# Bergvca/string_grouper

Hardware: AMD Instinct MI355X
Metric: hot-path rows/sec (the device path of match_strings: tokenise + tf-idf + postings + SpGEMM-topn, inputs resident in HBM), 663k-name self-join ntop=10 min_sim=0.8; match_strings end to end: match_strings_rows_per_s (higher is better)
Workload: dtype f32

## Files before the change

string_grouper_amd/csrc/sg_k4_device.h:

```cpp
#ifndef SG_K4_DEVICE_H
#define SG_K4_DEVICE_H
#include <math.h>

#include "sg_internal.h"

#define SG_TOPN_LANES 64

#ifdef SG_WATCHDOG
static __device__ int g_sg_watch[4];
#define SG_WD_DECL(c) int c = 0
#define SG_WD(c, limit, code)                                   \
    if (++(c) > (int)(limit) || ((volatile int *)g_sg_watch)[0]) { \
        if (((volatile int *)g_sg_watch)[0] == 0) {             \
            g_sg_watch[0] = (code);                             \
            g_sg_watch[1] = (int)(c);                           \
        }                                                       \
        break;                                                  \
    }
#ifndef SG_WATCH_NAME
#define SG_WATCH_NAME sg_debug_watch
#endif
extern "C" int SG_WATCH_NAME(int32_t *out4) {
    return hipMemcpyFromSymbol(out4, HIP_SYMBOL(g_sg_watch), 16) == hipSuccess ? 0 : 4;
}
// ... 45 lines not shown
    int c;
    __device__ __forceinline__ void clear() {
        s = -INFINITY;
        c = INT32_MAX;
    }
    __device__ __forceinline__ void insert(T ns, int nc, int lane) {
        const bool mine_first = (s > ns) || (s == ns && c < nc);
        const int pos = __popcll(__ballot(mine_first));
        if (pos >= SG_TOPN_LANES) return;
        const T us = __shfl_up(s, 1, 64);
        const int uc = __shfl_up(c, 1, 64);
        if (lane > pos) {
            s = us;
            c = uc;
        } else if (lane == pos) {
            s = ns;
            c = nc;
        }
    }
    __device__ __forceinline__ void insert_unique(T ns, int nc, int lane) {
        if (__ballot(c == nc) != 0) return;
        insert(ns, nc, lane);
    }
};

template <typename T>
struct TopListWide {
    TopList<T> lo, hi;
    __device__ __forceinline__ void clear() {
        lo.clear();
        hi.clear();
    }
    __device__ __forceinline__ void insert(T ns, int nc, int lane) {
        const bool mine_first = (lo.s > ns) || (lo.s == ns && lo.c < nc);
        const int pos = __popcll(__ballot(mine_first));
        if (pos >= SG_TOPN_LANES) {
            hi.insert(ns, nc, lane);
            return;
        }
        const T es = wave_read<T>(lo.s, SG_TOPN_LANES - 1);
        const int ec = wave_read<int>(lo.c, SG_TOPN_LANES - 1);
        lo.insert(ns, nc, lane);
        if (ec != INT32_MAX) hi.insert(es, ec, lane);
    }
    __device__ __forceinline__ void insert_unique(T ns, int nc, int lane) {
        if (__ballot(lo.c == nc || hi.c == nc) != 0) return;
        insert(ns, nc, lane);
    }
    __device__ __forceinline__ int count() const {
        return __popcll(__ballot(lo.c != INT32_MAX)) + __popcll(__ballot(hi.c != INT32_MAX));
    }
};

template <typename T>
struct Post;
template <>
struct Post<float> {
    typedef uint2 reg_t;
    static constexpr int STRIDE = 8;
    static __device__ __forceinline__ reg_t load(const char *vals, const char *, uint32_t seg_lo, uint32_t entry) {
        return *reinterpret_cast<const uint2 *>(vals + ((seg_lo + entry) << 3));
    }
    static __device__ __forceinline__ uint32_t slot(const reg_t &r) { return r.x; }
    static __device__ __forceinline__ float val(const reg_t &r) { return __uint_as_float(r.y); }
};
template <>
struct Post<double> {
    struct reg_t {
        uint32_t j;
        double v;
    };
    static constexpr int STRIDE = 8;
    static __device__ __forceinline__ reg_t load(const char *vals, const char *slots, uint32_t seg_lo, uint32_t entry) {
        reg_t r;
        r.j = *reinterpret_cast<const uint32_t *>(slots + ((seg_lo + entry) << 2));
        r.v = *reinterpret_cast<const double *>(vals + ((seg_lo + entry) << 3));
        return r;
    }
    static __device__ __forceinline__ uint32_t slot(const reg_t &r) { return r.j; }
    static __device__ __forceinline__ double val(const reg_t &r) { return r.v; }
};


__device__ __forceinline__ uint32_t next_row(uint32_t *row_counter, int lane) {
    uint32_t r = 0;
    if (lane == 0) r = __hip_atomic_fetch_add(row_counter, 1u, __ATOMIC_RELAXED, __HIP_MEMORY_SCOPE_AGENT);
    return (uint32_t)__builtin_amdgcn_readfirstlane((int)r);
}

#endif
```

string_grouper_amd/csrc/sg_spgemm_pruned.hip:

```cpp
#define SG_WATCH_NAME sg_debug_watch_pruned
#include "sg_k4_device.h"

#ifdef SG_DEBUG_WAVE_TIMES
__device__ unsigned long long sg_debug_wave_times[4 * 16384];
extern "C" int sg_debug_read_wave_times(unsigned long long *out, int clear) {
    if (hipMemcpyFromSymbol(out, HIP_SYMBOL(sg_debug_wave_times), sizeof(sg_debug_wave_times)) != hipSuccess) return 1;
    if (clear) {
        static unsigned long long zero[4 * 16384];
        if (hipMemcpyToSymbol(HIP_SYMBOL(sg_debug_wave_times), zero, sizeof(zero)) != hipSuccess) return 1;
    }
    return 0;
}
#endif

#ifndef SG_F64_STREAM_WAVES
#define SG_F64_STREAM_WAVES 4
#endif
#define SG_SCHED_FENCE() __builtin_amdgcn_sched_barrier(0)
#define SG_ROW_PARTS_LOG2 6
#define SG_ROW_PARTS 64u
#define SG_SURV_CAP 128

__device__ __forceinline__ uint64_t ballot64(bool p) { return __builtin_amdgcn_ballot_w64(p); }

// ... 402 lines not shown
    if ((uint32_t)lane < n_surv) {
        c0 = surv[lane];
        k0 = (uint32_t)lane < n_clean ||
             __hip_atomic_exchange(&dt[((uint32_t)c0 * 2654435761u) >> 25], (uint32_t)c0, __ATOMIC_RELAXED,
                                   __HIP_MEMORY_SCOPE_WORKGROUP) != (uint32_t)c0;
    }
    if ((uint32_t)lane + 64u < n_surv) {
        c1 = surv[lane + 64];
        k1 = (uint32_t)lane + 64u < n_clean ||
             __hip_atomic_exchange(&dt[((uint32_t)c1 * 2654435761u) >> 25], (uint32_t)c1, __ATOMIC_RELAXED,
                                   __HIP_MEMORY_SCOPE_WORKGROUP) != (uint32_t)c1;
    }
    const uint64_t f0 = ballot64(k0), f1 = ballot64(k1);
    const uint32_t n0 = (uint32_t)__popcll(f0);
    __builtin_amdgcn_wave_barrier();
    if (k0) surv[__popcll(f0 & lanes_below)] = c0;
    if (k1) surv[n0 + __popcll(f1 & lanes_below)] = c1;
    __builtin_amdgcn_wave_barrier();
    FlushOut<T> out;
    out.top = top;
    out.n_surv = (uint32_t)__builtin_amdgcn_readfirstlane((int)(n0 + (uint32_t)__popcll(f1)));
    if (out.n_surv >= 63u) {
        out.top = drain_survivors<T, SYM, TILE_LOG2, WIDE, true>(nnz, thr, row, sc, pairs, top, out.n_surv);
        const uint32_t scored = out.n_surv < 64u ? out.n_surv : 64u;
        out.n_surv = (out.n_surv - scored) | (scored << 16);
    }
    return out;
}

template <typename T, int TILE_LOG2>
__device__ __noinline__ void emit_part_matches(const SgPairSink *__restrict__ pairs, T s, int c, int cnt, uint32_t row_out) {
    constexpr int TILE = 1 << TILE_LOG2;
    int *surv = lds_object<int>(TILE * 2 + 512 + 1024);
    const int lane = threadIdx.x;
    if (cnt <= 0) return;
    uint32_t pos = (uint32_t)surv[SG_SURV_CAP - 1];
    const SgPairSink pv = load_launch_constants(pairs);
    const uint32_t pair_chunks = pv.chunks;
    if (pos == SG_PAIR_NO_CHUNK || (pos & 511u) + (uint32_t)cnt > SG_PAIR_CHUNK) {
        uint32_t ch = 0;
        if (lane == 0) {
            if (pos != SG_PAIR_NO_CHUNK && (pos >> 9) < pair_chunks) {
                pv.d_chunk_count[pos >> 9] = pos & 511u;
                atomicAdd(pv.d_totals, (unsigned long long)(pos & 511u));
            }
            ch = atomicAdd(pv.d_chunks_used, 1u);
        }
        pos = (uint32_t)__builtin_amdgcn_readfirstlane((int)ch) << 9;
    }
    if ((pos >> 9) < pair_chunks) {
        if (lane < cnt) {
            const size_t o = (size_t)(pos >> 9) * SG_PAIR_CHUNK + (pos & 511u) + (uint32_t)lane;
            pv.d_i[o] = (uint32_t)c;
            pv.d_j[o] = row_out;
            reinterpret_cast<T *>(pv.d_s)[o] = s;
        }
        if (lane == 0) atomicAdd(&pv.d_row_count[row_out], (uint32_t)cnt);
    }
    __builtin_amdgcn_wave_barrier();
    if (lane == 0) surv[SG_SURV_CAP - 1] = (int)(pos + (uint32_t)cnt);
}

template <typename T, int TILE_LOG2, bool SYM, bool WIDE, int FOLD_LOG2, bool SHARE = false>
__global__ void __launch_bounds__(64, (sizeof(T) == 8 && FOLD_LOG2 > 0) ? SG_F64_STREAM_WAVES : 4)
spgemm_topn_pruned_kernel(const int64_t *__restrict__ a_indptr, const int32_t *__restrict__ a_indices,
                          const T *__restrict__ a_data, uint32_t n_left, const uint32_t *__restrict__ seg,
                          const uint32_t *__restrict__ ends, int32_t nt_pad, uint32_t n_terms,
                          const uint32_t *__restrict__ filt, int32_t n_tiles,
                          const SgScoreCtx *__restrict__ sc ,
                          int32_t keep, int32_t out_stride, T thr,
                          float s_budget , float norm_b ,
                          uint32_t freq_min ,
                          int32_t *__restrict__ out_cols, T *__restrict__ out_vals, int32_t *__restrict__ out_cnt,
                          uint32_t *row_counter, uint32_t *flagged_count, uint32_t *flagged_rows,
                          unsigned long long *stats ,
                          const SgPairSink *__restrict__ pairs ,
                          uint32_t pair_chunks ,
                          uint32_t sym_lo, uint32_t sym_hi ,
                          const uint32_t *__restrict__ row_list , const uint32_t *row_list_len,
                          const uint32_t *__restrict__ ends8 , int32_t nv_pad,
                          uint32_t null_off ,
                          uint32_t n_right ,
                          uint32_t *heavy_count, uint32_t *heavy_rows ,
                          uint32_t sym_step,
                          uint32_t part_cfg ) {
    constexpr int TILE = 1 << TILE_LOG2;
    constexpr int SLOTS = WIDE ? 2 : 1;
    constexpr int AB = TILE_LOG2 + 1;
    constexpr uint32_t ADDR_MASK = ((1u << AB) - 1u) & ~3u;
    constexpr int FB = AB + FOLD_LOG2;
    constexpr uint32_t BQ_BITS = 24 - FB;
    constexpr uint32_t BQ_MAX = (1u << BQ_BITS) - 1u;
    constexpr float SCALE = (float)(32768 >> FOLD_LOG2);
    extern __shared__ __attribute__((aligned(16))) unsigned char smem[];
    int *hk = reinterpret_cast<int *>(smem + TILE * 2);
    T *ha = reinterpret_cast<T *>(smem + TILE * 2 + 512);
    int *surv = reinterpret_cast<int *>(smem + TILE * 2 + 512 + 1024);
    uint4 *tab_v = reinterpret_cast<uint4 *>(smem);
    const int lane = threadIdx.x;
    for (int x = lane; x < TILE * 2 / 16; x += 64) tab_v[x] = make_uint4(0, 0, 0, 0);
    if (SYM && lane == 0) surv[SG_SURV_CAP - 1] = (int)SG_PAIR_NO_CHUNK;
    if (FOLD_LOG2 > 0 && lane == 0) surv[SG_SURV_CAP - 2] = 0;
    const uint64_t lanes_below = (1ull << lane) - 1ull;
    unsigned long long st_rows = 0, st_post = 0, st_surv = 0;
    auto tab_at = [&](uint32_t byte_addr) {
        typedef __attribute__((address_space(3))) uint32_t lds_u32;
        return (uint32_t *)(lds_u32 *)(uintptr_t)byte_addr;
    };
    auto filt_at = [&](uint32_t byte_off) {
        return *reinterpret_cast<const uint32_t *>(reinterpret_cast<const char *>(filt) + byte_off);
    };

    SG_WD_DECL(wd_rows);
    constexpr bool CAN_SPLIT = SYM && !WIDE && FOLD_LOG2 > 0 && SHARE;
    const bool part_mode = CAN_SPLIT && (part_cfg >> 31) != 0u;
#ifdef SG_DEBUG_WAVE_TIMES
    const unsigned long long dbg_t0 = __builtin_amdgcn_s_memrealtime();
    unsigned long long dbg_worst = 0, dbg_worst_row = 0;
#endif
    const uint32_t n_here = (WIDE || part_mode) ? (uint32_t)__builtin_amdgcn_readfirstlane((int)*row_list_len) << (part_mode ? SG_ROW_PARTS_LOG2 : 0)
                                                : (SYM ? (sym_hi - sym_lo + sym_step - 1u) / sym_step : n_left);
    const uint32_t n_single = min(n_here, 2u * gridDim.x);
    const uint32_t n_quads = (n_here - n_single) >> 2;
    for (uint32_t hlp = next_row(row_counter, lane);; hlp = next_row(row_counter, lane)) {
    const uint32_t row0 = hlp < n_quads ? hlp << 2 : (n_quads << 2) + (hlp - n_quads);
    if (row0 >= n_here || hlp >= 0x10000000u) break;
    for (uint32_t rr = row0; rr < row0 + (hlp < n_quads ? 4u : 1u); ++rr) {
        SG_WD(wd_rows, n_left + 2, 11)
        const uint32_t row = WIDE ? (uint32_t)__builtin_amdgcn_readfirstlane((int)row_list[rr])
                                  : part_mode ? (uint32_t)__builtin_amdgcn_readfirstlane((int)row_list[rr >> SG_ROW_PARTS_LOG2])
                                              : (SYM ? sym_hi - 1u - rr * sym_step : rr);
        uint32_t part_lo = 0, part_hi = 0;
        if (CAN_SPLIT && part_mode) {
            const uint32_t from = (uint32_t)__builtin_amdgcn_readfirstlane((int)row_list[n_left + (rr >> SG_ROW_PARTS_LOG2)]);
            const uint32_t nv = (((row >> TILE_LOG2) + (1u << FOLD_LOG2)) >> FOLD_LOG2) - from;
            const uint32_t part = rr & (SG_ROW_PARTS - 1u);
            part_lo = from + ((part * nv) >> SG_ROW_PARTS_LOG2);
            part_hi = from + (((part + 1u) * nv) >> SG_ROW_PARTS_LOG2);
            if (part_lo == part_hi) continue;
        }
        uint32_t row_out = row;
        if (SYM) {
            const uint32_t *orig_of = sc->orig_of;
            if (orig_of) row_out = (uint32_t)__builtin_amdgcn_readfirstlane((int)orig_of[row]);
        }
        const int64_t rlo = a_indptr[row];
        const int nnz = __builtin_amdgcn_readfirstlane((int)(a_indptr[row + 1] - rlo));
        if (nnz > 64 * SLOTS) {
            if (lane == 0) flagged_rows[atomicAdd(flagged_count, 1u)] = row;
            continue;
        }
        if (nnz == 0) continue;
        int k[SLOTS];
        T a[SLOTS];
        uint32_t df[SLOTS], lo_e[SLOTS];
        float w[SLOTS], cum[SLOTS];
#pragma unroll
        for (int sl = 0; sl < SLOTS; ++sl) {
            k[sl] = 0;
            a[sl] = (T)0;
            df[sl] = lo_e[sl] = 0;
            if (lane + 64 * sl < nnz) {
                k[sl] = a_indices[rlo + lane + 64 * sl];
                a[sl] = a_data[rlo + lane + 64 * sl];
                const uint32_t *sp = seg + (int64_t)k[sl] * n_tiles;
                lo_e[sl] = sp[0];
                df[sl] = sp[n_tiles] - lo_e[sl];
            }
            w[sl] = lane + 64 * sl < nnz ? (float)a[sl] * (float)a[sl] * 1.00001f : 0.f;
            cum[sl] = 0.f;
        }
        for (int q = 0; q < nnz; ++q) {
            uint32_t dq;
            float wq;
            if (SLOTS == 1 || q < 64) {
                dq = wave_read<uint32_t>(df[0], q);
                wq = wave_read<float>(w[0], q);
            } else {
                dq = wave_read<uint32_t>(df[SLOTS - 1], q - 64);
                wq = wave_read<float>(w[SLOTS - 1], q - 64);
            }
#pragma unroll
            for (int sl = 0; sl < SLOTS; ++sl) {
                const bool before = dq > df[sl] || (dq == df[sl] && q <= lane + 64 * sl);
                cum[sl] += before ? wq : 0.f;
            }
        }
        bool in_p[SLOTS];
        uint64_t pm[SLOTS];
        float bs2 = 0.f, dsum = 0.f;
        int np = 0;
#pragma unroll
        for (int sl = 0; sl < SLOTS; ++sl) {
            const bool have = lane + 64 * sl < nnz;
            const bool in_s = have && cum[sl] <= s_budget && df[sl] >= freq_min;
            in_p[sl] = have && !in_s;
            pm[sl] = __ballot(in_p[sl]);
            np += __popcll(pm[sl]);
            bs2 = fmaxf(bs2, in_s ? cum[sl] : 0.f);
            dsum += in_p[sl] ? (float)df[sl] : 0.f;
        }
        if (np == 0) continue;
        if (np > 64) {
            if (lane == 0) flagged_rows[atomicAdd(flagged_count, 1u)] = row;
            continue;
        }
        if (!part_mode) ++st_rows;
#ifdef SG_DEBUG_WAVE_TIMES
        const unsigned long long dbg_r0 = __builtin_amdgcn_s_memrealtime();
        const unsigned long long dbg_surv0 = st_surv;
#endif
#pragma unroll
        for (int d = 32; d > 0; d >>= 1) {
            bs2 = fmaxf(bs2, __shfl_xor(bs2, d, 64));
            dsum += __shfl_xor(dsum, d, 64);
        }
        bs2 = wave_read<float>(bs2, 0);
        dsum = wave_read<float>(dsum, 0);
        if (!(dsum > 0.f)) continue;
        const float b_s = sqrtf(bs2) * 1.000002f;
        const float t0 = ((float)thr - 1e-5f) * SCALE - 2.0f;
        const float c1 = b_s * norm_b * (SCALE / 255.0f) * 1.000002f;
        const int32_t T0 = (int32_t)floorf(t0 * 256.0f) - 256 * np;
        const int32_t C1 = (int32_t)(c1 * 256.0f) + 1;
        const int32_t C16 = (int32_t)(b_s * norm_b * (SCALE * 65536.0f / 65280.0f) * 1.000002f) + 1;
        const int32_t T16 = T0 << 8;
        const int32_t T0s = T16 - 32768 * C16, C1n = -C16;
        if (FOLD_LOG2 > 0 ? !(T16 - C16 * 65535 >= 65536) : !(T0 - C1 * 255 >= 256)) {
            if (lane == 0) flagged_rows[atomicAdd(flagged_count, 1u)] = row;
            continue;
        }
        const int32_t T0m = T0 - 256;

        uint32_t G[SLOTS], start[SLOTS];
        uint32_t before_slot = 0;
#pragma unroll
        for (int sl = 0; sl < SLOTS; ++sl) {
            G[sl] = in_p[sl] ? 1u + (uint32_t)((float)(64 - np) * 0.999f * ((float)df[sl] / dsum)) : 0u;
            uint32_t inc = G[sl];
#pragma unroll
            for (int d = 1; d < 64; d <<= 1) {
                const uint32_t o = __shfl_up(inc, d, 64);
                if (lane >= d) inc += o;
            }
            start[sl] = before_slot + inc - G[sl];
            before_slot += wave_read<uint32_t>(inc, 63);
        }
        int src = 0, src_slot = 0;
        uint32_t u = 0, g = 0;
#pragma unroll
        for (int sl = 0; sl < SLOTS; ++sl) {
            uint64_t m = pm[sl];
            SG_WD_DECL(wd_a);
            while (m) {
                SG_WD(wd_a, 70, 12)
                const int f = __builtin_ctzll(m);
                m &= m - 1;
                const uint32_t sf = wave_read<uint32_t>(start[sl], f), gf = wave_read<uint32_t>(G[sl], f);
                const uint32_t d = (uint32_t)lane - sf;
                if (d < gf) {
                    src = f;
                    src_slot = sl;
                    u = d;
                    g = gf;
                }
            }
        }
        int my_k = wave_shfl<int>(k[0], src);
        uint32_t my_lo = wave_shfl<uint32_t>(lo_e[0], src);
        T my_a = wave_shfl<T>(a[0], src);
        if (SLOTS > 1) {
            const int k1 = wave_shfl<int>(k[SLOTS - 1], src);
            const uint32_t lo1 = wave_shfl<uint32_t>(lo_e[SLOTS - 1], src);
            const T a1 = wave_shfl<T>(a[SLOTS - 1], src);
            if (src_slot) {
                my_k = k1;
                my_lo = lo1;
                my_a = a1;
            }
        }
        const float c_a = (float)my_a * norm_b * (SCALE / (float)BQ_MAX) * 1.000002f;
        const uint32_t CA = (uint32_t)(c_a * (float)(1u << (32 - FB))) + 1u;
        const uint32_t u4 = u << 2, u16 = u << 4, G4 = g << 2, G16 = g << 4;
        const int32_t over16 = (int32_t)(G16 - u16);
        const uint32_t erow = (g ? (uint32_t)my_k : n_terms) * (uint32_t)nt_pad;
        auto ends_at = [&](uint32_t group) {
            return *reinterpret_cast<const uint4 *>(reinterpret_cast<const char *>(ends) + ((erow + (group << 2)) << 2));
        };
        const uint32_t t_end = SYM ? (row >> TILE_LOG2) + 1u : (uint32_t)n_tiles;
        const uint32_t last_group = (uint32_t)(nt_pad >> 2) - 1u;

        if (WIDE) {
#pragma unroll
            for (int sl = 0; sl < SLOTS; ++sl) {
                hk[lane + 64 * sl] = lane + 64 * sl < nnz ? k[sl] : INT32_MAX;
                ha[lane + 64 * sl] = a[sl];
            }
            __builtin_amdgcn_wave_barrier();
        } else {
            hk[lane] = -1;
            hk[lane + 64] = -1;
            __builtin_amdgcn_wave_barrier();
            if (lane < nnz) {
                uint32_t h = term_hash(k[0]);
                SG_WD_DECL(wd_i);
                while (atomicCAS(&hk[h], -1, k[0]) != -1) {
                    SG_WD(wd_i, SG_HASH_SLOTS + 2, 16)
                    h = (h + 1) & (SG_HASH_SLOTS - 1);
                }
                ha[h] = a[0];
            }
            __builtin_amdgcn_wave_barrier();
        }

        TopList<T> top;
        top.clear();
        uint32_t n_surv = 0;
        uint32_t row_arg = row | ((SYM && keep > SG_TOPN_LANES) ? 0x40000000u : 0u);
        if (SYM && FOLD_LOG2 > 0 && !part_mode) {
            T own = (T)0;
            for (int q = 0; q < nnz; ++q) {
                const T aq = (SLOTS == 1 || q < 64) ? wave_read<T>(a[0], q) : wave_read<T>(a[SLOTS - 1], q - 64);
                own = add_rn<T>(own, mul_rn<T>(aq, aq));
            }
            if (own > thr) top.insert(own, (int)row_out, lane);
            row_arg |= 0x80000000u;
        }

        auto collect = [&](uint64_t cm, uint32_t r, uint32_t t) {
            bool cross = (cm >> lane) & 1ull;
            const int col = (int)((t << TILE_LOG2) | ((r & ADDR_MASK) >> 1) | (r & 1u));
            if (SYM) {
                cross = cross && (uint32_t)col <= row;
                cm = ballot64(cross);
            }
            if (cross) surv[n_surv + __popcll(cm & lanes_below)] = col;
            n_surv += __popcll(cm);
            if (n_surv >= 64) {
                top = drain_survivors<T, SYM, TILE_LOG2, WIDE, (FOLD_LOG2 > 0)>(nnz, thr, row_arg, sc, pairs, top, n_surv);
                st_surv += 64;
                n_surv -= 64;
            }
        };
        auto round = [&](uint32_t r, bool valid, uint64_t valid_mask, uint32_t t, uint32_t &zaddr) {
            zaddr = r & ADDR_MASK;
            const uint32_t sh = r << 4;
            const uint32_t x = (uint32_t)(((uint64_t)(r & (BQ_MAX << FB)) * (uint64_t)(CA & 0xffffffu)) >> 32);
            const uint32_t tq1 = (uint32_t)((T0m - __mul24(C1, (int32_t)(r >> 24))) >> 8);
            uint32_t xs;
            asm("v_lshlrev_b32 %0, %1, %2" : "=v"(xs) : "v"(sh), "v"(x));
            uint32_t old;
            asm("" : "=v"(old));
            if (valid)
                old = __hip_atomic_fetch_add(tab_at(zaddr), xs, __ATOMIC_RELAXED, __HIP_MEMORY_SCOPE_WORKGROUP);
            asm volatile("" : "+v"(old));
            const uint32_t oh = __builtin_amdgcn_ubfe(old, sh, 16u);
            const uint64_t cm = ballot64(tq1 - oh < x) & valid_mask;
            if (cm) collect(cm, r, t);
        };

        struct Batch {
            uint32_t r0, r1, r2, r3;
            int32_t rem;
            uint32_t base;
        };
        auto issue = [&](Batch &bt, uint32_t lo, uint32_t hi) {
            bt.base = lo + u16;
            bt.rem = (int32_t)(hi - bt.base);
            struct __attribute__((packed, aligned(4))) Quad {
                uint32_t x, y, z, w;
            };
            const Quad q = *reinterpret_cast<const Quad *>(reinterpret_cast<const char *>(filt) + bt.base);
            bt.r0 = q.x;
            bt.r1 = q.y;
            bt.r2 = q.z;
            bt.r3 = q.w;
        };
        struct Slot {
            uint32_t z, sh, x, xs, tq1;
        };
        auto prep = [&](uint32_t r) {
            Slot s;
            s.z = r & ADDR_MASK;
            s.sh = r << 4;
            s.x = (uint32_t)(((uint64_t)(r & (BQ_MAX << FB)) * (uint64_t)(CA & 0xffffffu)) >> 32);
            s.tq1 = (uint32_t)((T0m - __mul24(C1, (int32_t)(r >> 24))) >> 8);
            asm("v_lshlrev_b32 %0, %1, %2" : "=v"(s.xs) : "v"(s.sh), "v"(s.x));
            return s;
        };
        auto apply = [&](const Batch &bt, uint32_t t) {
            const bool v0 = bt.rem > 0, v1 = bt.rem > 4, v2 = bt.rem > 8, v3 = bt.rem > 12;
            const uint64_t m0 = ballot64(v0), m1 = ballot64(v1), m2 = ballot64(v2), m3 = ballot64(v3);
            if (m0 == 0) return;
            if (ballot64(bt.rem > over16)) {
                uint32_t zz = 0;
                round(bt.r0, v0, m0, t, zz);
                round(bt.r1, v1, m1, t, zz);
                round(bt.r2, v2, m2, t, zz);
                round(bt.r3, v3, m3, t, zz);
                int32_t left = bt.rem - over16 - (int32_t)u4;
                uint32_t at = bt.base + (uint32_t)over16 + u4;
                SG_WD_DECL(wd_b);
                uint64_t ml;
                while ((ml = ballot64(left > 0)) != 0) {
                    SG_WD(wd_b, 1 << 24, 14)
                    const uint32_t rx = filt_at(at);
                    round(rx, left > 0, ml, t, zz);
// ... 258 lines not shown
                apply_s(sb2, sb3, sb0, sb1, tv2, la2);
                issue_s(sb2, tv2, la2);
                if (tv3 >= v_end) break;
                apply_s(sb3, sb0, sb1, sb2, tv3, la3);
                issue_s(sb3, tv3, la3);
            }
            asm volatile("s_waitcnt vmcnt(0) ; rounds %0 %1 %2 %3 ends %4 %5" : "+v"(sb0.q), "+v"(sb1.q), "+v"(sb2.q), "+v"(sb3.q), "+v"(EA), "+v"(EB)::"memory");
            if (n_surv > n_clean) flush_s(sb1, sb2, sb3, v_end);
            if (CAN_SPLIT && !part_mode && v_end != n_visits && lane == 0) {
                const uint32_t at = atomicAdd(heavy_count, 1u);
                heavy_rows[at] = row;
                heavy_rows[n_left + at] = v_end;
            }
        }
        {
            uint32_t mine = 0;
            if (g && u == 0 && part_lo == 0u) {
                const uint32_t *erp = ends + (size_t)erow;
                mine = (erp[t_end - 1u] >> 2) - my_lo;
            }
#pragma unroll
            for (int d = 32; d > 0; d >>= 1) mine += __shfl_xor(mine, d, 64);
            st_post += (unsigned long long)wave_read<uint32_t>(mine, 0);
        }
        if (n_surv > 0) {
            top = drain_survivors<T, SYM, TILE_LOG2, WIDE, (FOLD_LOG2 > 0)>(nnz, thr, row_arg, sc, pairs, top, n_surv);
            st_surv += n_surv;
        }
        if (CAN_SPLIT && part_mode) {
            int cnt = __popcll(__ballot(top.c != INT32_MAX));
            if (cnt > keep) cnt = keep;
            emit_part_matches<T, TILE_LOG2>(pairs, top.s, top.c, cnt, row_out);
        } else {
            int cnt = __popcll(__ballot(top.c != INT32_MAX));
            if (cnt > keep) cnt = keep;
            const size_t obase = (size_t)row_out * (size_t)out_stride;
            if (lane < cnt) {
                out_vals[obase + lane] = top.s;
                out_cols[obase + lane] = top.c;
            }
            if (lane == 0) out_cnt[row_out] = cnt;
        }
        if (SYM) {
            const uint32_t pos = (uint32_t)__builtin_amdgcn_readfirstlane(surv[SG_SURV_CAP - 1]);
            if (pos != SG_PAIR_NO_CHUNK && (pos >> 9) >= pair_chunks && lane == 0) atomicMax(row_counter, 0x20000000u);
        }
#ifdef SG_DEBUG_WAVE_TIMES
        {
            const unsigned long long dt = __builtin_amdgcn_s_memrealtime() - dbg_r0;
            if (dt > dbg_worst) {
                dbg_worst = dt;
                dbg_worst_row = (unsigned long long)row | ((st_surv - dbg_surv0) << 32);
            }
        }
#endif
    }
    }
    if (SYM && lane == 0) {
        const uint32_t pos = (uint32_t)surv[SG_SURV_CAP - 1];
        if (pos != SG_PAIR_NO_CHUNK && (pos >> 9) < pair_chunks) {
            pairs->d_chunk_count[pos >> 9] = pos & 511u;
            atomicAdd(pairs->d_totals, (unsigned long long)(pos & 511u));
        }
    }
    if (lane == 0) {
        if (st_rows) atomicAdd(stats + 0, st_rows);
        if (st_post) atomicAdd(stats + 1, st_post);
        if (st_surv) atomicAdd(stats + 2, st_surv);
        if (FOLD_LOG2 > 0) {
            if (surv[SG_SURV_CAP - 2]) atomicAdd(stats + 4, (unsigned long long)(uint32_t)surv[SG_SURV_CAP - 2]);
        } else if (st_surv) atomicAdd(stats + 4, st_surv);
    }
#ifdef SG_DEBUG_WAVE_TIMES
    if (SYM && !WIDE && FOLD_LOG2 > 0 && sizeof(T) == 4 && lane == 0 && blockIdx.x < 8192u) {
        unsigned long long *w = sg_debug_wave_times + 4u * (blockIdx.x + (part_mode ? 8192u : 0u));
        w[0] = dbg_t0;
        w[1] = __builtin_amdgcn_s_memrealtime();
        w[2] = dbg_worst;
        w[3] = dbg_worst_row;
    }
#endif
}

__device__ __forceinline__ void publish_pass_stats(const unsigned long long *src, const uint32_t *word, unsigned long long *dst) {
    if (dst != nullptr && blockIdx.x == 0 && threadIdx.x == 0) {
        dst[0] = src[0];
        dst[1] = src[1];
        dst[2] = src[2];
        dst[4] = src[4];
        reinterpret_cast<uint32_t *>(dst + 3)[0] = *word;
    }
}

template <typename T>
__global__ void __launch_bounds__(SG_PAIR_CHUNK) pairs_fill_kernel(const uint32_t *__restrict__ pi, const uint32_t *__restrict__ pj,
                                                                   const T *__restrict__ ps, const uint32_t *__restrict__ chunk_count,
                                                                   const uint32_t *__restrict__ ptr, uint32_t *cursor,
                                                                   int32_t *__restrict__ lcol, T *__restrict__ lval) {
    if (threadIdx.x >= chunk_count[blockIdx.x]) return;
    const size_t p = (size_t)blockIdx.x * SG_PAIR_CHUNK + threadIdx.x;
    const uint32_t j = pj[p];
    const uint32_t at = ptr[j] + atomicAdd(&cursor[j], 1u);
    lcol[at] = (int32_t)pi[p];
    lval[at] = ps[p];
}

template <typename T>
__global__ void __launch_bounds__(SG_PAIR_CHUNK) pairs_export_kernel(const uint32_t *__restrict__ pi, const uint32_t *__restrict__ pj,
                                                                     const T *__restrict__ ps, const uint32_t *__restrict__ chunk_count,
                                                                     const uint32_t *__restrict__ chunk_start, int32_t *__restrict__ out,
                                                                     const unsigned long long *st_src, const uint32_t *st_word,
                                                                     unsigned long long *st_dst) {
    constexpr int W = sizeof(T) == 8 ? 4 : 3;
    publish_pass_stats(st_src, st_word, st_dst);
    if (threadIdx.x >= chunk_count[blockIdx.x]) return;
    const size_t p = (size_t)blockIdx.x * SG_PAIR_CHUNK + threadIdx.x;
    int32_t *o = out + ((size_t)chunk_start[blockIdx.x] + threadIdx.x) * W;
    o[0] = (int32_t)pi[p];
    o[1] = (int32_t)pj[p];
    if (sizeof(T) == 8) {
        const long long b = __double_as_longlong((double)ps[p]);
        o[2] = (int32_t)(b & 0xffffffffll);
        o[3] = (int32_t)(b >> 32);
    } else {
        o[2] = __float_as_int((float)ps[p]);
    }
}

template <int W>
__global__ void __launch_bounds__(256) pairs_flat_count_kernel(const int32_t *__restrict__ pairs, int64_t n_pairs, uint32_t lo,
                                                               uint32_t hi, uint32_t step, const uint32_t *__restrict__ pos_of,
                                                               uint32_t *cnt) {
    const int64_t p = (int64_t)blockIdx.x * blockDim.x + threadIdx.x;
    if (p >= n_pairs) return;
    const uint32_t j = (uint32_t)pairs[p * W + 1];
    const uint32_t at = pos_of ? pos_of[j] : j;
    if (at >= lo && at < hi && (hi - 1u - at) % step == 0u) atomicAdd(&cnt[j], 1u);
}

template <typename T>
__global__ void __launch_bounds__(256) pairs_flat_fill_kernel(const int32_t *__restrict__ pairs, int64_t n_pairs, uint32_t lo,
                                                              uint32_t hi, uint32_t step, const uint32_t *__restrict__ pos_of,
                                                              const uint32_t *__restrict__ ptr, uint32_t *cursor,
                                                              int32_t *__restrict__ lcol, T *__restrict__ lval) {
    constexpr int W = sizeof(T) == 8 ? 4 : 3;
    const int64_t p = (int64_t)blockIdx.x * blockDim.x + threadIdx.x;
    if (p >= n_pairs) return;
    const int32_t *rec = pairs + p * W;
    const uint32_t j = (uint32_t)rec[1];
    const uint32_t pj = pos_of ? pos_of[j] : j;
    if (pj < lo || pj >= hi || (hi - 1u - pj) % step != 0u) return;
    const uint32_t at = ptr[j] + atomicAdd(&cursor[j], 1u);
    lcol[at] = rec[0];
    if (sizeof(T) == 8)
        lval[at] = (T)__longlong_as_double(((long long)rec[3] << 32) | (long long)(uint32_t)rec[2]);
    else
        lval[at] = (T)__int_as_float(rec[2]);
}

template <typename T>
__global__ void __launch_bounds__(64) pairs_select_kernel(const uint32_t *__restrict__ ptr, const int32_t *__restrict__ lcol,
                                                          const T *__restrict__ lval, uint32_t n_rows, int32_t keep,
                                                          int32_t out_stride, int32_t *__restrict__ out_cols,
                                                          T *__restrict__ out_vals, int32_t *__restrict__ out_cnt,
                                                          const unsigned long long *st_src, const uint32_t *st_word,
                                                          unsigned long long *st_dst) {
// ... 222 lines not shown
struct PairList {
    SgPairSink sink;
    const SgPairSink *d_sink = nullptr;
    uint32_t row_lo = 0, row_hi = 0;
    uint32_t row_step = 1;
    uint32_t rows() const { return (row_hi - row_lo + row_step - 1u) / row_step; }
};

__global__ void pair_sink_kernel(SgPairSink v, SgPairSink *out) { *out = v; }

bool sg_q8_applies(const sg_ctx *ctx, const sg_postings *Bt, double threshold) {
    if (!Bt->d_q8 || Bt->fold_log2 <= 0) return false;
    return threshold >= ctx->opt_double("SG_Q8_MIN_THRESHOLD", 0.65);
}

static size_t pruned_lds(int32_t tile_log2, int32_t fold_log2, int32_t dtype) {
    return ((size_t)2 << tile_log2) + 512 + 1024 + (size_t)SG_SURV_CAP * 4 + (fold_log2 > 0 && dtype == SG_F64 ? 512 : 0);
}
static unsigned pruned_grid(const sg_ctx *ctx, int32_t tile_log2, int64_t n_rows, int32_t fold_log2 = 0, int32_t dtype = SG_F32) {
    const size_t lds = pruned_lds(tile_log2, fold_log2, dtype);
    int waves_per_cu = (int)(ctx->lds_per_cu / lds);
    if (waves_per_cu > 32) waves_per_cu = 32;
    if (waves_per_cu < 1) waves_per_cu = 1;
    const int forced = ctx->opt_int("SG_PRUNE_WAVES_PER_CU", 0);
    if (forced > 0) waves_per_cu = forced;
    unsigned grid = (unsigned)ctx->num_cu * (unsigned)waves_per_cu;
    if ((int64_t)grid > n_rows) grid = (unsigned)(n_rows > 0 ? n_rows : 1);
    return grid;
}

struct PrunedJob {
    sg_ctx *ctx;
    const sg_csr *A;
    const sg_postings *Bt;
    int32_t keep;
    sg_topn *r;
    double threshold;
    float s_budget;
    unsigned long long *stats = nullptr;
    uint32_t *row_counter = nullptr;
    uint32_t *flagged_count = nullptr, *flagged_rows = nullptr;
    const PairList *pl = nullptr;
};

struct PrunedLaunch {
    uint32_t *row_counter;
    uint32_t *out_count, *out_rows;
    const uint32_t *in_rows = nullptr, *in_len = nullptr;
    uint32_t *heavy_count = nullptr, *heavy_rows = nullptr;
    uint32_t part_cfg = 0;
};

struct RowList {
    uint32_t *base = nullptr;
    uint32_t *count() const { return base; }
    uint32_t *counter() const { return base ? base + 1 : nullptr; }
    uint32_t *rows() const { return base ? base + 4 : nullptr; }
};

template <typename T, int TILE_LOG2, bool SYM, bool WIDE, int FOLD_LOG2>
static int launch_pruned(const PrunedJob &job, const PrunedLaunch &l) {
    sg_ctx *ctx = job.ctx;
    const sg_csr *A = job.A;
    const sg_postings *Bt = job.Bt;
    const sg_topn *r = job.r;
    const PairList &pl = *job.pl;
    const T thr = (T)job.threshold;
    const size_t lds = pruned_lds(TILE_LOG2, FOLD_LOG2, A->dtype);
    unsigned grid = pruned_grid(ctx, TILE_LOG2, SYM ? (int64_t)pl.rows() : A->n_rows, FOLD_LOG2, A->dtype);
    if (WIDE && grid > (unsigned)ctx->num_cu * 4u && (double)A->nnz <= 48.0 * (double)A->n_rows) grid = (unsigned)ctx->num_cu * 4u;
    constexpr bool SPLITS = SYM && !WIDE && FOLD_LOG2 > 0;
    const bool share = SPLITS && (l.heavy_count != nullptr || l.part_cfg != 0u);
    auto kernel = share ? spgemm_topn_pruned_kernel<T, TILE_LOG2, SYM, WIDE, FOLD_LOG2, SPLITS>
                        : spgemm_topn_pruned_kernel<T, TILE_LOG2, SYM, WIDE, FOLD_LOG2, false>;
    hipLaunchKernelGGL(kernel, dim3(grid), dim3(64), lds, ctx->stream, A->d_indptr,
                       A->d_indices, (const T *)A->d_data, (uint32_t)A->n_rows, (const uint32_t *)Bt->d_seg,
                       (const uint32_t *)Bt->d_ends, Bt->nt_pad, (uint32_t)Bt->n_terms,
                       (const uint32_t *)Bt->d_filt, Bt->n_tiles,
                       (const SgScoreCtx *)Bt->d_score_ctx + (sg_q8_applies(ctx, Bt, (double)thr) ? 0 : 1), job.keep, r->stride, thr,
                       job.s_budget, Bt->norm_up, Bt->freq_min, r->d_cols,
                       (T *)r->d_vals,
                       r->d_counts, l.row_counter, l.out_count, l.out_rows, job.stats, pl.d_sink, pl.sink.chunks, pl.row_lo, pl.row_hi,
                       l.in_rows, l.in_len, (const uint32_t *)Bt->d_ends8, Bt->nv_pad, (uint32_t)(Bt->nnz * 4), (uint32_t)Bt->n_right,
                       l.heavy_count, l.heavy_rows, pl.row_step, l.part_cfg);
    SG_HIP_TRY(hipGetLastError());
    return SG_OK;
}

static uint32_t heavy_part_cfg(const sg_ctx *ctx, const sg_csr *A, const PairList &range, int32_t tile_log2, int32_t fold_log2) {
    uint32_t heavy_rounds = 0;
    if ((range.row_lo > 0 || (int64_t)range.row_hi < A->n_rows || range.row_step > 1) && 2 * (int64_t)range.rows() < A->n_rows) {
        const double n_idx = (double)A->n_rows;
        const double rows_per_wave = (double)range.rows() / (double)pruned_grid(ctx, tile_log2, (int64_t)range.rows(), fold_log2, A->dtype);
        const double rounds_per_row = 2.0 * 7.2e-5 * n_idx * (0.5 * ((double)range.row_lo + (double)range.row_hi) / n_idx);
        const double share = ctx->opt_double("SG_HEAVY_SHARE", 0.0);
        const double bar_share = share > 0.0 ? share : 0.05;
        const double bar = bar_share * rows_per_wave * rounds_per_row;
        heavy_rounds = bar < 128.0 ? 128u : (bar > 1.0e9 ? 1000000000u : (uint32_t)bar);
    }
    heavy_rounds = (uint32_t)ctx->opt_int("SG_HEAVY_ROUNDS", (int)heavy_rounds) & 0x7fffffffu;
    if (heavy_rounds > 0x0fffffffu) heavy_rounds = 0x0fffffffu;
    uint32_t handover_shift = heavy_rounds >= 512u ? 1u : (heavy_rounds >= 256u ? 2u : 3u);
    handover_shift = (uint32_t)ctx->opt_int("SG_HANDOVER_SHIFT", (int)handover_shift) & 7u;
    if (heavy_rounds) heavy_rounds |= handover_shift << 28;
    return heavy_rounds;
}

template <typename T, int TILE_LOG2, bool SYM, int FOLD_LOG2>
static int launch_both(const PrunedJob &job) {
    sg_ctx *ctx = job.ctx;
    const int64_t n_rows = job.A->n_rows;
    Scratch scratch(ctx);
    RowList l1, heavy;
    SG_TRY(scratch.alloc((size_t)n_rows + 8, &l1.base));
    if (hipMemsetAsync(l1.base, 0, 4 * sizeof(uint32_t), ctx->stream) != hipSuccess) return SG_ERR_HIP;
    uint32_t part_cfg = 0;
    if (SYM && FOLD_LOG2 > 0) part_cfg = heavy_part_cfg(ctx, job.A, *job.pl, TILE_LOG2, FOLD_LOG2);
    if (part_cfg) {
        SG_TRY(scratch.alloc(2 * (size_t)n_rows + 8, &heavy.base));
        if (hipMemsetAsync(heavy.base, 0, 4 * sizeof(uint32_t), ctx->stream) != hipSuccess) return SG_ERR_HIP;
    }
    const PrunedLaunch first{job.row_counter, l1.count(), l1.rows(), nullptr, nullptr, heavy.count(), heavy.rows(), part_cfg};
    SG_TRY((launch_pruned<T, TILE_LOG2, SYM, false, FOLD_LOG2>(job, first)));
    if (heavy.base) {
        const PrunedLaunch parts{heavy.counter(), l1.count(), l1.rows(), heavy.rows(), heavy.count(), nullptr, nullptr, 0x80000000u};
        SG_TRY((launch_pruned<T, TILE_LOG2, SYM, false, FOLD_LOG2>(job, parts)));
        scratch.release(heavy.base);
    }
    if (!ctx->opt_is("SG_PRUNE_WIDE", '0')) {
        const PrunedLaunch wide{l1.counter(), job.flagged_count, job.flagged_rows, l1.rows(), l1.count()};
        return launch_pruned<T, TILE_LOG2, SYM, true, FOLD_LOG2>(job, wide);
    }
    if (hipMemcpyAsync(job.flagged_count, l1.count(), 4, hipMemcpyDeviceToDevice, ctx->stream) != hipSuccess ||
        hipMemcpyAsync(job.flagged_rows, l1.rows(), sizeof(uint32_t) * (size_t)n_rows, hipMemcpyDeviceToDevice, ctx->stream) != hipSuccess)
        return SG_ERR_HIP;
    return SG_OK;
}

template <typename T, bool SYM>
static int dispatch_pruned(const PrunedJob &job) {
    const sg_postings *Bt = job.Bt;
    if (Bt->fold_log2 > 0) {
        if (Bt->fold_log2 != 3 || Bt->tile_log2 != 12 || !Bt->d_ends8) {
            sg_set_error("postings folded 2^%d over tiles of 2^%d columns are not supported by the pruned multiply", Bt->fold_log2,
                         Bt->tile_log2);
            return SG_ERR_UNSUPPORTED;
        }
        return launch_both<T, 12, SYM, 3>(job);
    }
    switch (Bt->tile_log2) {
        case 11: return launch_both<T, 11, SYM, 0>(job);
        case 12: return launch_both<T, 12, SYM, 0>(job);
        case 13: return launch_both<T, 13, SYM, 0>(job);
        default:
            sg_set_error("postings tile of 2^%d columns is not supported by the pruned multiply (2^11..2^13)", Bt->tile_log2);
            return SG_ERR_UNSUPPORTED;
    }
}

bool sg_pruned_supports_tile(int32_t tile_log2) { return tile_log2 >= 11 && tile_log2 <= 13; }

static float prune_budget(const sg_postings *Bt, double threshold, double delta) {
    const double nb = (double)Bt->norm_up;
    const double beta = threshold - delta;
    const double budget = (beta / nb) * (beta / nb) * (1.0 - 1e-6);
    return __builtin_nextafterf((float)budget, 0.f);
}
// ... 280 lines not shown
```

Measured before the change: 104.3 million.

## Deal lanes by largest-remainder share and rank only frequent terms via packed keys

Per-row lane allocation moves from a float floor-rule with a prefix-scan of start offsets to an integer largest-remainder split. The split finds its remainder cutoff by binary search over ballots, so all 64 lanes are handed out. The cumulative-weight ranking now packs df and lane into one sortable key and loops only over terms with df ≥ freq_min (via a ballot mask) rather than all nnz. The self-norm sum is folded into that loop. The aim is fewer wave_read iterations in the per-row setup and fuller lane use in the streaming phase. The trade-off is extra integer division and ballot work, plus possible changes in pruning bounds from the new ordering and skipped terms.

```diff
diff --git a/string_grouper_amd/csrc/sg_k4_device.h b/string_grouper_amd/csrc/sg_k4_device.h
--- a/string_grouper_amd/csrc/sg_k4_device.h
+++ b/string_grouper_amd/csrc/sg_k4_device.h
@@ -151,6 +151,48 @@
 };
 
 
+template <typename U>
+__host__ __device__ __forceinline__ void sg_deal_share(U df, U dsum, uint32_t spare, uint32_t &q, U &rem) {
+    if constexpr (sizeof(U) == 8) {
+        const U num = (U)spare * df;
+        q = (uint32_t)(num / dsum);
+        rem = num % dsum;
+    } else {
+#ifdef __HIP_DEVICE_COMPILE__
+        const float inv = __builtin_amdgcn_rcpf((float)dsum);
+#else
+        const float inv = 1.0f / (float)dsum;
+#endif
+        q = (uint32_t)((float)spare * (float)df * inv);
+        int32_t r = (int32_t)(spare * df - q * dsum);
+        if (r < 0) {
+            --q;
+            r += (int32_t)dsum;
+        } else if (r >= (int32_t)dsum) {
+            ++q;
+            r -= (int32_t)dsum;
+        }
+        rem = (U)r;
+    }
+}
+template <typename U, typename AtLeast>
+__host__ __device__ __forceinline__ U sg_deal_cut(U dsum, uint32_t R, AtLeast at_least) {
+    U cut = 0;
+    if (dsum < 2) return cut;
+    const int top = (sizeof(U) == 8 ? 63 - __builtin_clzll((unsigned long long)(dsum - 1)) : 31 - __builtin_clz((unsigned)(dsum - 1)));
+    for (U bit = (U)1 << top; bit; bit >>= 1) {
+        const uint32_t n = at_least(cut | bit);
+        if (n >= R) {
+            cut |= bit;
+            if (n == R) break;
+        }
+    }
+    return cut;
+}
+__host__ __device__ __forceinline__ uint32_t sg_deal_floor_rule(uint32_t df, float dsum, int np) {
+    return 1u + (uint32_t)((float)(64 - np) * 0.999f * ((float)df / dsum));
+}
+
 __device__ __forceinline__ uint32_t next_row(uint32_t *row_counter, int lane) {
     uint32_t r = 0;
     if (lane == 0) r = __hip_atomic_fetch_add(row_counter, 1u, __ATOMIC_RELAXED, __HIP_MEMORY_SCOPE_AGENT);
diff --git a/string_grouper_amd/csrc/sg_spgemm_pruned.hip b/string_grouper_amd/csrc/sg_spgemm_pruned.hip
--- a/string_grouper_amd/csrc/sg_spgemm_pruned.hip
+++ b/string_grouper_amd/csrc/sg_spgemm_pruned.hip
@@ -508,7 +508,7 @@
                           uint32_t null_off ,
                           uint32_t n_right ,
                           uint32_t *heavy_count, uint32_t *heavy_rows ,
-                          uint32_t sym_step,
+                          uint32_t sym_step, uint32_t deal_floor ,
                           uint32_t part_cfg ) {
     constexpr int TILE = 1 << TILE_LOG2;
     constexpr int SLOTS = WIDE ? 2 : 1;
@@ -578,43 +578,63 @@
         }
         if (nnz == 0) continue;
         int k[SLOTS];
-        T a[SLOTS];
-        uint32_t df[SLOTS], lo_e[SLOTS];
+        T a[SLOTS], a2[SLOTS];
+        uint32_t df[SLOTS], lo_e[SLOTS], key[SLOTS];
         float w[SLOTS], cum[SLOTS];
+        uint64_t fm[SLOTS];
 #pragma unroll
         for (int sl = 0; sl < SLOTS; ++sl) {
             k[sl] = 0;
             a[sl] = (T)0;
             df[sl] = lo_e[sl] = 0;
-            if (lane + 64 * sl < nnz) {
+            const bool have = lane + 64 * sl < nnz;
+            if (have) {
                 k[sl] = a_indices[rlo + lane + 64 * sl];
                 a[sl] = a_data[rlo + lane + 64 * sl];
                 const uint32_t *sp = seg + (int64_t)k[sl] * n_tiles;
                 lo_e[sl] = sp[0];
                 df[sl] = sp[n_tiles] - lo_e[sl];
             }
-            w[sl] = lane + 64 * sl < nnz ? (float)a[sl] * (float)a[sl] * 1.00001f : 0.f;
+            a2[sl] = mul_rn<T>(a[sl], a[sl]);
+            w[sl] = have ? (sizeof(T) == 4 ? (float)a2[sl] : (float)a[sl] * (float)a[sl]) * 1.00001f : 0.f;
             cum[sl] = 0.f;
-        }
-        for (int q = 0; q < nnz; ++q) {
-            uint32_t dq;
-            float wq;
-            if (SLOTS == 1 || q < 64) {
-                dq = wave_read<uint32_t>(df[0], q);
-                wq = wave_read<float>(w[0], q);
-            } else {
-                dq = wave_read<uint32_t>(df[SLOTS - 1], q - 64);
-                wq = wave_read<float>(w[SLOTS - 1], q - 64);
-            }
-#pragma unroll
-            for (int sl = 0; sl < SLOTS; ++sl) {
-                const bool before = dq > df[sl] || (dq == df[sl] && q <= lane + 64 * sl);
-                cum[sl] += before ? wq : 0.f;
+            key[sl] = (min(df[sl], (1u << 25) - 1u) << 7) | (127u - (uint32_t)(lane + 64 * sl));
+            fm[sl] = ballot64(have && df[sl] >= freq_min);
+        }
+        const bool sum_own = SYM && FOLD_LOG2 > 0 && !part_mode;
+        T own = (T)0;
+        auto rank_step = [&](int sl_q, int f) {
+            const uint32_t kq = wave_read<uint32_t>(key[sl_q], f);
+            const float wq = wave_read<float>(w[sl_q], f);
+#pragma unroll
+            for (int sl = 0; sl < SLOTS; ++sl) cum[sl] += kq >= key[sl] ? wq : 0.f;
+        };
+        if (sum_own) {
+#pragma unroll
+            for (int sl_q = 0; sl_q < SLOTS; ++sl_q) {
+                const int n_q = min(nnz - 64 * sl_q, 64);
+                for (int f = 0; f < n_q; ++f) {
+                    own = add_rn<T>(own, wave_read<T>(a2[sl_q], f));
+                    if ((fm[sl_q] >> f) & 1ull) rank_step(sl_q, f);
+                }
+            }
+        } else {
+#pragma unroll
+            for (int sl_q = 0; sl_q < SLOTS; ++sl_q) {
+                uint64_t m = fm[sl_q];
+                SG_WD_DECL(wd_r);
+                while (m) {
+                    SG_WD(wd_r, 70, 18)
+                    const int f = __builtin_ctzll(m);
+                    m &= m - 1;
+                    rank_step(sl_q, f);
+                }
             }
         }
         bool in_p[SLOTS];
         uint64_t pm[SLOTS];
-        float bs2 = 0.f, dsum = 0.f;
+        float bs2 = 0.f;
+        uint32_t dsum_i = 0;
         int np = 0;
 #pragma unroll
         for (int sl = 0; sl < SLOTS; ++sl) {
@@ -624,7 +644,7 @@
             pm[sl] = __ballot(in_p[sl]);
             np += __popcll(pm[sl]);
             bs2 = fmaxf(bs2, in_s ? cum[sl] : 0.f);
-            dsum += in_p[sl] ? (float)df[sl] : 0.f;
+            dsum_i += in_p[sl] ? df[sl] : 0u;
         }
         if (np == 0) continue;
         if (np > 64) {
@@ -639,11 +659,11 @@
 #pragma unroll
         for (int d = 32; d > 0; d >>= 1) {
             bs2 = fmaxf(bs2, __shfl_xor(bs2, d, 64));
-            dsum += __shfl_xor(dsum, d, 64);
+            dsum_i += __shfl_xor(dsum_i, d, 64);
         }
         bs2 = wave_read<float>(bs2, 0);
-        dsum = wave_read<float>(dsum, 0);
-        if (!(dsum > 0.f)) continue;
+        dsum_i = wave_read<uint32_t>(dsum_i, 0);
+        if (dsum_i == 0u) continue;
         const float b_s = sqrtf(bs2) * 1.000002f;
         const float t0 = ((float)thr - 1e-5f) * SCALE - 2.0f;
         const float c1 = b_s * norm_b * (SCALE / 255.0f) * 1.000002f;
@@ -658,22 +678,55 @@
         }
         const int32_t T0m = T0 - 256;
 
-        uint32_t G[SLOTS], start[SLOTS];
-        uint32_t before_slot = 0;
+        uint32_t G[SLOTS], rem[SLOTS];
 #pragma unroll
         for (int sl = 0; sl < SLOTS; ++sl) {
-            G[sl] = in_p[sl] ? 1u + (uint32_t)((float)(64 - np) * 0.999f * ((float)df[sl] / dsum)) : 0u;
-            uint32_t inc = G[sl];
-#pragma unroll
-            for (int d = 1; d < 64; d <<= 1) {
-                const uint32_t o = __shfl_up(inc, d, 64);
-                if (lane >= d) inc += o;
-            }
-            start[sl] = before_slot + inc - G[sl];
-            before_slot += wave_read<uint32_t>(inc, 63);
+            rem[sl] = 0u;
+            if (deal_floor) {
+                G[sl] = in_p[sl] ? sg_deal_floor_rule(df[sl], (float)dsum_i, np) : 0u;
+            } else {
+                uint32_t q = 0;
+                sg_deal_share<uint32_t>(in_p[sl] ? df[sl] : 0u, dsum_i, (uint32_t)(64 - np), q, rem[sl]);
+                G[sl] = in_p[sl] ? 1u + q : 0u;
+            }
+        }
+        if (!deal_floor) {
+            uint32_t given = 0;
+#pragma unroll
+            for (int sl = 0; sl < SLOTS; ++sl) {
+                uint64_t m = pm[sl];
+                SG_WD_DECL(wd_g);
+                while (m) {
+                    SG_WD(wd_g, 70, 19)
+                    given += wave_read<uint32_t>(G[sl], __builtin_ctzll(m));
+                    m &= m - 1;
+                }
+            }
+            if (given < 64u) {
+                const uint32_t R = 64u - given;
+                const uint32_t cut = sg_deal_cut<uint32_t>(dsum_i, R, [&](uint32_t c) {
+                    uint32_t n = 0;
+#pragma unroll
+                    for (int sl = 0; sl < SLOTS; ++sl) n += (uint32_t)__popcll(ballot64(rem[sl] >= c));
+                    return n;
+                });
+                auto below = [](uint64_t m) { return __builtin_amdgcn_mbcnt_hi((uint32_t)(m >> 32), __builtin_amdgcn_mbcnt_lo((uint32_t)m, 0u)); };
+                uint32_t n_above = 0;
+#pragma unroll
+                for (int sl = 0; sl < SLOTS; ++sl) n_above += (uint32_t)__popcll(ballot64(rem[sl] > cut));
+                uint32_t at_before = 0;
+#pragma unroll
+                for (int sl = 0; sl < SLOTS; ++sl) {
+                    const bool at = in_p[sl] && rem[sl] == cut;
+                    const uint64_t am = ballot64(at);
+                    G[sl] += (rem[sl] > cut || (at && at_before + below(am) < R - n_above)) ? 1u : 0u;
+                    at_before += (uint32_t)__popcll(am);
+                }
+            }
         }
         int src = 0, src_slot = 0;
         uint32_t u = 0, g = 0;
+        uint32_t first_lane = 0;
 #pragma unroll
         for (int sl = 0; sl < SLOTS; ++sl) {
             uint64_t m = pm[sl];
@@ -682,14 +735,15 @@
                 SG_WD(wd_a, 70, 12)
                 const int f = __builtin_ctzll(m);
                 m &= m - 1;
-                const uint32_t sf = wave_read<uint32_t>(start[sl], f), gf = wave_read<uint32_t>(G[sl], f);
-                const uint32_t d = (uint32_t)lane - sf;
+                const uint32_t gf = wave_read<uint32_t>(G[sl], f);
+                const uint32_t d = (uint32_t)lane - first_lane;
                 if (d < gf) {
                     src = f;
                     src_slot = sl;
                     u = d;
                     g = gf;
                 }
+                first_lane += gf;
             }
         }
         int my_k = wave_shfl<int>(k[0], src);
@@ -743,12 +797,7 @@
         top.clear();
         uint32_t n_surv = 0;
         uint32_t row_arg = row | ((SYM && keep > SG_TOPN_LANES) ? 0x40000000u : 0u);
-        if (SYM && FOLD_LOG2 > 0 && !part_mode) {
-            T own = (T)0;
-            for (int q = 0; q < nnz; ++q) {
-                const T aq = (SLOTS == 1 || q < 64) ? wave_read<T>(a[0], q) : wave_read<T>(a[SLOTS - 1], q - 64);
-                own = add_rn<T>(own, mul_rn<T>(aq, aq));
-            }
+        if (sum_own) {
             if (own > thr) top.insert(own, (int)row_out, lane);
             row_arg |= 0x80000000u;
         }
@@ -1173,6 +1222,51 @@
 #endif
 }
 
+extern "C" int sg_debug_deal_lanes(const uint32_t *df, int np, uint32_t *G_out, int floor_rule) {
+    if (np < 1 || np > 64 || !df || !G_out) return 1;
+    uint64_t dsum = 0;
+    for (int t = 0; t < np; ++t) dsum += df[t];
+    if (dsum == 0) return 1;
+    if (floor_rule) {
+        for (int t = 0; t < np; ++t) G_out[t] = sg_deal_floor_rule(df[t], (float)dsum, np);
+        return 0;
+    }
+    const uint32_t spare = (uint32_t)(64 - np);
+    uint64_t rem[64];
+    uint32_t given = 0;
+    for (int t = 0; t < np; ++t) {
+        uint32_t q = 0;
+        sg_deal_share<uint64_t>(df[t], dsum, spare, q, rem[t]);
+        if (dsum < (1ull << 30)) {
+            uint32_t q32 = 0, rem32 = 0;
+            sg_deal_share<uint32_t>(df[t], (uint32_t)dsum, spare, q32, rem32);
+            if (q32 != q || rem32 != rem[t]) return 2;
+        }
+        G_out[t] = 1u + q;
+        given += G_out[t];
+    }
+    if (given < 64u) {
+        const uint32_t R = 64u - given;
+        const uint64_t cut = sg_deal_cut<uint64_t>(dsum, R, [&](uint64_t c) {
+            uint32_t n = 0;
+            for (int t = 0; t < np; ++t) n += rem[t] >= c ? 1u : 0u;
+            return n;
+        });
+        uint32_t left = R;
+        for (int t = 0; t < np; ++t)
+            if (rem[t] > cut) {
+                ++G_out[t];
+                --left;
+            }
+        for (int t = 0; t < np && left; ++t)
+            if (rem[t] == cut) {
+                ++G_out[t];
+                --left;
+            }
+    }
+    return 0;
+}
+
 __device__ __forceinline__ void publish_pass_stats(const unsigned long long *src, const uint32_t *word, unsigned long long *dst) {
     if (dst != nullptr && blockIdx.x == 0 && threadIdx.x == 0) {
         dst[0] = src[0];
@@ -1561,7 +1655,7 @@
                        (T *)r->d_vals,
                        r->d_counts, l.row_counter, l.out_count, l.out_rows, job.stats, pl.d_sink, pl.sink.chunks, pl.row_lo, pl.row_hi,
                        l.in_rows, l.in_len, (const uint32_t *)Bt->d_ends8, Bt->nv_pad, (uint32_t)(Bt->nnz * 4), (uint32_t)Bt->n_right,
-                       l.heavy_count, l.heavy_rows, pl.row_step, l.part_cfg);
+                       l.heavy_count, l.heavy_rows, pl.row_step, ctx->opt_is("SG_DEAL", 'f') ? 1u : 0u, l.part_cfg);
     SG_HIP_TRY(hipGetLastError());
     return SG_OK;
 }
```

Result: faster. 106.8 million (median of 6 runs) (+2.4%).
